# sloisel/MultiGridBarrierMPI.jl

Hardware: AMD Instinct MI355X
Metric: fem2d p-Laplace DoF/s per Newton step (higher is better)
Workload: dtype f64; 1 GPU; fem2d p-Laplace L=7 p=1 (n=57344 rows, N_L=49154 Newton unknowns), amgb main phase, tol=sqrt(eps); parallelism=single GPU

## Files before the change

multigridbarriermpi.jl_amd/csrc/gpuchol.hip:

```cpp
#include "gpuchol.hpp"

#include "amg.hpp"

#include <algorithm>
#include <array>
#include <cmath>
#include <cstdio>
#include <cstdlib>
#include <stdexcept>
#include <string>

namespace mgb {

namespace {

void ck(hipError_t e, const char* what) {
  if (e != hipSuccess) throw HipError(std::string("HIP error in gpuchol ") + what + ": " + hipGetErrorString(e));
}

constexpr int kProfSlots = 10;
#ifdef MGB_PROF_LAST_WG
#define MGB_PROF_WG (gridDim.x - 1)
#else
#define MGB_PROF_WG 0
// ... 980 lines not shown
      src[u] = (k < t.a1) ? asm_src[k] : 0;
    }
#pragma unroll
    for (int u = 0; u < 4; ++u) v[u] = vals[src[u]];
#pragma unroll
    for (int u = 0; u < 4; ++u) add_entry(pos[u], v[u]);
  }
  if (prm >= 0) ATI[tid * TP + nf - r0] += bval;
  __syncthreads();
  factor_diag_block<NARROW, DENSE>(D, kw, Lo, (t.ti == 0 && t.tj == 0) ? linv + t.loff : nullptr, fail, nullptr);
  if (!DENSE) {
    for (int idx = tid; idx < PB * PB; idx += TB) Lc[lq_index(idx % PB, idx / PB)] = Lo[(idx % PB) * LP + idx / PB];
    __syncthreads();
  }
  STAMP(2);
  const double* Lf = DENSE ? Lo : Lc;
  if (diag) trsm_block64<NARROW, DENSE>(ATI, TP, Lf, kw);
  else trsm_block64_pair<NARROW, DENSE>(ATI, ATJ, TP, Lf, kw);
  __syncthreads();
  if (t.tj == min((int)t.ti, max(1, (nf - k1 + TS - 1) / TS) - 1)) {
    for (int idx = tid; idx < TS * PB; idx += TB) {
      const int r = idx / PB, m = idx % PB;
      if (r0 + r <= nf && m < kw) F[(long long)ld * (r0 + r) + m] = ATI[m * TP + r];
    }
  }
  STAMP(3);
  if (PRE && DENSE) {
#pragma unroll
    for (int bj = 0; bj < 4; ++bj)
#pragma unroll
      for (int reg = 0; reg < 4; ++reg) {
        const int i = r0 + 16 * w + li, j = c0 + 16 * bj + lk + 4 * reg;
        c[bj][reg] = slab(i <= nf && j < nf && i >= j, i, j);
      }
  }
  typedef double v4f64 __attribute__((ext_vector_type(4)));
  const double* LI = ATI + 16 * w + li + lk * TP;
  const double* LJ = (diag ? ATI : ATJ) + li + lk * TP;
  v4f64 acc[4];
#pragma unroll
  for (int bj = 0; bj < 4; ++bj) acc[bj] = v4f64{c[bj][0], c[bj][1], c[bj][2], c[bj][3]};
#pragma unroll
  for (int ks = 0; ks < (NARROW ? 2 : PB / 4); ++ks) {
    const double bv = -LI[4 * ks * TP];
#pragma unroll
    for (int bj = 0; bj < 4; ++bj)
      acc[bj] = __builtin_amdgcn_mfma_f64_16x16x4f64(LJ[4 * ks * TP + 16 * bj], bv, acc[bj], 0, 0, 0);
  }
  double* E = slabs + (producer ? t.eoff : 0);
  const int* fwJ = rowJ[0];
  const int fi = producer ? rowI[0][16 * w + li] : 0;
#pragma unroll
  for (int bj = 0; bj < 4; ++bj)
#pragma unroll
    for (int reg = 0; reg < 4; ++reg) {
      const int i = r0 + 16 * w + li, j = c0 + 16 * bj + lk + 4 * reg;
      if (i <= nf && j < nf && i >= j) {
        if (producer) E[(long long)t.pld * fwJ[16 * bj + lk + 4 * reg] + fi] = acc[bj][reg];
        else F[(long long)ld * j + i] = acc[bj][reg];
      }
    }
  STAMP(7);
}

template <bool NARROW, bool PRE>
__global__ __launch_bounds__(TB) __attribute__((amdgpu_waves_per_eu(2, 2))) void front_single_kernel(
    const SingleTile* __restrict__ tiles, const int* __restrict__ pinv, const int* __restrict__ asm_src,
    const int* __restrict__ asm_pos, const double* __restrict__ vals, const int* __restrict__ perm, const double* __restrict__ b,
    const double* __restrict__ fronts_ro, double* fronts, double* linv, int* fail, long long* prof,
    const double* __restrict__ slabs_ro, double* slabs, const int* __restrict__ fwd) {
  front_single_body<NARROW, false, PRE>(tiles, pinv, asm_src, asm_pos, vals, perm, b, fronts_ro, fronts, linv, fail, prof, slabs_ro,
                                        slabs, fwd);
}

template <bool NARROW, bool PRE>
__global__ __launch_bounds__(TB) __attribute__((amdgpu_waves_per_eu(3, 3))) void front_single_dense_kernel(
    const SingleTile* __restrict__ tiles, const int* __restrict__ pinv, const int* __restrict__ asm_src,
    const int* __restrict__ asm_pos, const double* __restrict__ vals, const int* __restrict__ perm, const double* __restrict__ b,
    const double* __restrict__ fronts_ro, double* fronts, double* linv, int* fail, long long* prof,
    const double* __restrict__ slabs_ro, double* slabs, const int* __restrict__ fwd) {
  front_single_body<NARROW, true, PRE>(tiles, pinv, asm_src, asm_pos, vals, perm, b, fronts_ro, fronts, linv, fail, prof, slabs_ro,
                                       slabs, fwd);
}

__global__ __launch_bounds__(TB, 4) void front_leaf_kernel(
    const GNode* __restrict__ nodes, const int* __restrict__ list, const int* __restrict__ asm_src,
    const int* __restrict__ asm_pos, const double* __restrict__ vals, const int* __restrict__ perm,
    const double* __restrict__ b, double* fronts, double* linv, int* fail, long long* prof, double* slabs,
    const int* __restrict__ fwd) {
  extern __shared__ __attribute__((aligned(32))) double sm[];
  __shared__ int fw[TS];
  STAMP(0);
  const GNode nd = nodes[blockIdx.x];
  (void)list;
  const int nf = nd.nf, ld = nf + 1, ns = nd.ns, tid = threadIdx.x;
  const bool producer = nd.eoff >= 0;
  if (producer && tid <= nf - ns && tid < TS) fw[tid] = fwd[nd.fofs + tid];
  constexpr int TP = TS + 8;
  __shared__ __attribute__((aligned(32))) double fixed[TP * PB + PB * (PB + 1) / 2];
  double* Fs = sm;
  double* AT = fixed;
  double* D = fixed;
  double* Lo = fixed + TP * PB;
  auto P = [ld](int i, int j) { return j * ld - (j * (j - 1)) / 2 + (i - j); };
  const int total = nf * ld - (nf * (nf - 1)) / 2;
  double* F = fronts + nd.off;
  for (int idx = tid; idx < total; idx += TB) Fs[idx] = 0.0;
  __syncthreads();
  for (int k = nd.a0 + tid; k < nd.a1; k += TB) {
    const int pos = asm_pos[k], col = pos / ld;
    Fs[P(pos - col * ld, col)] += vals[asm_src[k]];
  }
  for (int c = tid; c < ns; c += TB) Fs[P(nf, c)] += b[perm[nd.first + c]];
  __syncthreads();
  STAMP(1);
  auto panel = [&](const int p) {
    const int k0 = p * PB, kw = min(PB, ns - k0), k1 = k0 + kw;
    for (int idx = tid; idx < PB * PB; idx += TB) {
      const int i = idx % PB, j = idx / PB;
      D[i * LP + j] = (i < kw && j <= i) ? Fs[P(k0 + i, k0 + j)] : 0.0;
    }
    __syncthreads();
    factor_diag_block<true, true>(D, kw, Lo, linv + nd.loff + (long long)p * 2 * PB * PB, fail, nullptr);
    for (int idx = tid; idx < TS * PB; idx += TB) {
      const int r = idx % TS, q = idx / TS;
      AT[q * TP + r] = (q < kw && k1 + r <= nf) ? Fs[P(k1 + r, k0 + q)] : 0.0;
    }
    __syncthreads();
    trsm_block64<true, true>(AT, TP, Lo, kw);
    __syncthreads();
    for (int idx = tid; idx < TS * PB; idx += TB) {
      const int r = idx / PB, m = idx % PB;
      if (k1 + r <= nf && m < kw) F[(long long)ld * (k1 + r) + k0 + m] = AT[m * TP + r];
    }
    typedef double v4f64 __attribute__((ext_vector_type(4)));
    const int lane = tid & 63, w = tid >> 6, li = lane & 15, lk = lane >> 4;
    const double* LI = AT + 16 * w + li + lk * TP;
    const double* LJ = AT + li + lk * TP;
    v4f64 acc[4];
#pragma unroll
    for (int bj = 0; bj < 4; ++bj) acc[bj] = v4f64{0.0, 0.0, 0.0, 0.0};
#pragma unroll 1
    for (int ks = 0; ks < (kw + 3) / 4; ++ks) {
      const double bv = LI[4 * ks * TP];
#pragma unroll
      for (int bj = 0; bj < 4; ++bj)
        acc[bj] = __builtin_amdgcn_mfma_f64_16x16x4f64(LJ[4 * ks * TP + 16 * bj], bv, acc[bj], 0, 0, 0);
    }
#pragma unroll
    for (int bj = 0; bj < 4; ++bj)
#pragma unroll
      for (int reg = 0; reg < 4; ++reg) {
        const int i = k1 + 16 * w + li, j = k1 + 16 * bj + lk + 4 * reg;
        if (i <= nf && j < nf && i >= j) Fs[P(i, j)] -= acc[bj][reg];
      }
    __syncthreads();
  };
  panel(0);
  if (ns > PB) panel(1);
  STAMP(2);
  const int nb = nf - ns;
  if (producer) {
    double* E = slabs + nd.eoff;
    for (int idx = tid; idx < (nb + 1) * nb; idx += TB) {
      const int a = idx % (nb + 1), q = idx / (nb + 1);
      if (a >= q) E[(long long)nd.pld * fw[q] + fw[a]] = Fs[P(ns + a, ns + q)];
    }
  } else {
    for (int idx = tid; idx < (nb + 1) * nb; idx += TB) {
      const int i = ns + idx % (nb + 1), j = ns + idx / (nb + 1);
      if (i >= j) F[(long long)ld * j + i] = Fs[P(i, j)];
    }
  }
  STAMP(7);
}

template <int NT>
__device__ inline void rect_part(const double* __restrict__ F, int ld, int ns, int nb, int j0, int jw,
                                 const double* xb, double* red, double* out , bool subtract) {
  const int tid = threadIdx.x;
  const int nsl = NT / jw, jl = tid % jw, sl = tid / jw, j = j0 + jl;
  double s = 0.0;
  if (sl < nsl && j < ns) {
    const double* col = F + (long long)ld * ns + j;
#pragma unroll 8
    for (int i = sl; i < nb; i += nsl) s = fma(col[(long long)ld * i], xb[i], s);
  }
  if (nsl > 1) {
    red[tid] = s;
    __syncthreads();
    if (sl == 0)
      for (int q = 1; q < nsl; ++q) s += red[q * jw + jl];
  }
  if (sl == 0 && j < ns) out[j] = subtract ? out[j] - s : s;
}

__global__ __launch_bounds__(RT) void backward_rect_kernel(const GNode* __restrict__ nodes, const RectJob* __restrict__ jobs,
                                                            const int* __restrict__ bdry_all,
                                                            const double* __restrict__ fronts, const double* __restrict__ y,
                                                            double* rect) {
  extern __shared__ double sh[];
  const RectJob job = jobs[blockIdx.x];
  const GNode nd = nodes[blockIdx.x];
  const int nf = nd.nf, ns = nd.ns, nb = nf - ns;
  const int* bd = bdry_all + nd.bofs;
  double* xb = sh;
  double* red = sh + nb;
  for (int i = threadIdx.x; i < nb; i += RT) xb[i] = y[bd[i]];
  __syncthreads();
  rect_part<RT>(fronts + nd.off, nf + 1, ns, nb, job.chunk * 64, 64, xb, red, rect + nd.first, false);
}

template <int NT>
__global__ __launch_bounds__(NT) void backward_kernel(const GNode* __restrict__ nodes, const int* __restrict__ list,
                                                       const int* __restrict__ bdry_all, const double* __restrict__ fronts,
                                                       const double* __restrict__ linv, const int* __restrict__ perm,
                                                       const double* __restrict__ rect, int use_rect, double* y, double* x,
                                                       long long* prof) {
  extern __shared__ double sh[];
  STAMP(0);
  const GNode nd = nodes[blockIdx.x];
  (void)list;
  const int nf = nd.nf, ns = nd.ns, nb = nf - ns, ld = nf + 1, tid = threadIdx.x;
  const double* F = fronts + nd.off;
  double* u = sh;
  double* xb = sh + ns;
  double* red = sh + nf;
  for (int i = tid; i < ns; i += NT) u[i] = F[(long long)ld * nf + i] - ((use_rect && nb > 0) ? rect[nd.first + i] : 0.0);
  STAMP(1);
  if (!use_rect && nb > 0) {
    const int* bd = bdry_all + nd.bofs;
    for (int i = tid; i < nb; i += NT) xb[i] = y[bd[i]];
    __syncthreads();
    const int jw = min(NT, (ns + 63) & ~63);
    for (int j0 = 0; j0 < ns; j0 += jw) {
      rect_part<NT>(F, ld, ns, nb, j0, jw, xb, red, u, true);
      __syncthreads();
    }
  }
  __syncthreads();
  STAMP(2);
  const int npanel = (ns + PB - 1) / PB;
  for (int pp = npanel - 1; pp >= 0; --pp) {
    const int k0 = pp * PB, kw = min(PB, ns - k0), k1 = k0 + kw;
    if (tid < 64) {
      const int c = tid & 31;
      const double* lpp = linv + nd.loff + (long long)pp * 2 * PB * PB + c;
      double lc[PB];
#pragma unroll
      for (int m = 0; m < PB; ++m) lc[m] = lpp[PB * m];
      double uc = (c < kw) ? u[k0 + c] : 0.0;
#pragma unroll
      for (int m = PB - 1; m >= 0; --m) {
        const double xm = readlane_f64(uc * lc[m], m);
        uc = (c == m) ? xm : fma(-lc[m], xm, uc);
      }
      if (tid < kw) u[k0 + c] = uc;
      if (pp == npanel - 1) STAMP(3);
    }
    __syncthreads();
    if (pp == npanel - 1) STAMP(4);
    if (k0 > 0) {
      const int jw = min(NT, (k0 + 63) & ~63), nsl = NT / jw;
      for (int jb = 0; jb < k0; jb += jw) {
        const int jl = tid % jw, sl = tid / jw, j = jb + jl;
        double s = 0.0;
        if (sl < nsl && j < k0) {
#pragma unroll 8
          for (int i = k0 + sl; i < k1; i += nsl) s = fma(F[(long long)ld * i + j], u[i], s);
        }
        if (nsl > 1) {
          red[tid] = s;
          __syncthreads();
          if (sl == 0)
            for (int q = 1; q < nsl; ++q) s += red[q * jw + jl];
        }
        if (sl == 0 && j < k0) u[j] -= s;
      }
      __syncthreads();
    }
    if (pp == npanel - 1) STAMP(5);
  }
  STAMP(6);
  for (int i = tid; i < ns; i += NT) {
    const double v = u[i];
    y[nd.first + i] = v;
    x[perm[nd.first + i]] = v;
  }
  STAMP(7);
}


__device__ __forceinline__ void load_pivot_block(double (&lc)[PB], const double* __restrict__ lpp, int lane) {
#pragma unroll
  for (int m = 0; m < PB; ++m) lc[m] = lpp[PB * m + (lane & 31)];
}

__device__ __forceinline__ void load_panel_rows(double (&f)[PB], const double* __restrict__ F, int ld, int k0, int kw, int jc) {
  const double* Fj = F + (long long)ld * k0 + max(min(jc, k0 - 1), 0);
#pragma unroll
  for (int r = 0; r < PB; ++r) f[r] = Fj[(long long)ld * min(r, kw - 1)];
}

__device__ __forceinline__ void panel_substitute(const double (&lc)[PB], double* up, int kw, int lane) {
  const int c = lane & 31;
  double uc = (c < kw) ? up[c] : 0.0;
#pragma unroll
  for (int m = PB - 1; m >= 0; --m) {
    const double xm = readlane_f64(uc * lc[m], m);
    uc = (c == m) ? xm : fma(-lc[m], xm, uc);
  }
  if (lane < kw) up[c] = uc;
}

template <int NSL>
__device__ __forceinline__ double panel_dot(const double (&f)[PB], const double* up, int kw) {
  double s[NSL];
#pragma unroll
  for (int q = 0; q < NSL; ++q) s[q] = 0.0;
#pragma unroll
  for (int r = 0; r < PB; ++r) {
    const double v = fma(f[r], up[min(r, kw - 1)], s[r % NSL]);
    s[r % NSL] = (r < kw) ? v : s[r % NSL];
  }
  double t = s[0];
#pragma unroll
  for (int q = 1; q < NSL; ++q) t += s[q];
  return t;
}

__device__ inline double panel_dot_any(const double* __restrict__ Fj, long long ld, const double* up, int kw, int nsl) {
  double t = 0.0;
  for (int q = 0; q < nsl; ++q) {
    double s = 0.0;
    for (int r = q; r < kw; r += nsl) s = fma(Fj[ld * r], up[r], s);
    t = q ? t + s : s;
  }
  return t;
}

__device__ __forceinline__ int uni(int v) { return __builtin_amdgcn_readfirstlane(v); }

__global__ __launch_bounds__(512) void backward_fused_kernel(const int* __restrict__ wgs, int wstride, int max_levels, int xs_cap,
                                                              int red_cap, const int* __restrict__ slots,
                                                              const double* __restrict__ fronts, const double* __restrict__ linv,
                                                              const int* __restrict__ perm, double* y, double* x, long long* prof) {
  extern __shared__ double sh[];
  STAMP(0);
  int* rec = (int*)sh;
  double* xs = sh + wstride / 2;
  double* red = xs + xs_cap;
  int* sl = (int*)(red + red_cap);
  const int tid = threadIdx.x, T = blockDim.x, W = T >> 6, wave = uni(tid >> 6), lane = tid & 63;
  {
    const int* src = wgs + (size_t)blockIdx.x * wstride;
    for (int i = tid; i < wstride; i += T) rec[i] = src[i];
  }
  __syncthreads();
  const int nlevels = rec[0], njobs = rec[1], first_lv = rec[2], sub_lv = rec[5];
  const int* jobs = rec + kFusedHdr + kFusedLevelInts * max_levels;
  for (int jb = wave; jb < njobs; jb += W) {
    const int* j = jobs + kFusedJobInts * jb;
    const int nf = uni(j[FJ_NF]), ns = uni(j[FJ_NS]), flags = uni(j[FJ_FLAGS]), base = uni(j[FJ_BASE]);
    const long long off = ((long long)uni(j[FJ_OFF + 1]) << 32) | (unsigned)uni(j[FJ_OFF]);
    const double* srcv = (flags & 2) ? y + uni(j[FJ_FIRST]) : fronts + off + (long long)(nf + 1) * nf;
    for (int i0 = 0; i0 < ns; i0 += 256) {
      double v[4];
#pragma unroll
      for (int k = 0; k < 4; ++k) {
        const int i = i0 + 64 * k + lane;
        v[k] = srcv[min(i, ns - 1)];
      }
#pragma unroll
      for (int k = 0; k < 4; ++k) {
        const int i = i0 + 64 * k + lane;
        if (i < ns) xs[base + i] = v[k];
      }
    }
    if (flags & 2) continue;
    const int nb = nf - ns;
    const int* ssrc = slots + uni(j[FJ_SOFS]);
    int* sdst = sl + uni(j[FJ_LSOFS]);
    for (int i0 = 0; i0 < nb; i0 += 256) {
      int v[4];
#pragma unroll
      for (int k = 0; k < 4; ++k) {
        const int i = i0 + 64 * k + lane;
        v[k] = ssrc[min(i, nb - 1)];
      }
#pragma unroll
      for (int k = 0; k < 4; ++k) {
        const int i = i0 + 64 * k + lane;
        if (i < nb) sdst[i] = v[k];
      }
    }
  }
  __syncthreads();
  STAMP(1);
  if (first_lv == sub_lv) STAMP(2);
  for (int lv = first_lv; lv < nlevels; ++lv) {
    const int* li = rec + kFusedHdr + kFusedLevelInts * lv;
    const int lofs = li[0], cnt = li[1], maxp = li[2], items = li[3];
    int G = W;
    while (G > 1 && W / G < cnt) G >>= 1;
    const int ngrp = W / G, GT = G << 6, grp = wave / G, gtid = tid - grp * GT, gw = wave - grp * G;
    double* redg = red + grp * items;
    for (int r0 = 0; r0 < cnt; r0 += ngrp) {
      const bool act = r0 + grp < cnt;
      const int* j = jobs + kFusedJobInts * (lofs + (act ? r0 + grp : 0));
      const int nf = uni(j[FJ_NF]), ns = uni(j[FJ_NS]), nsl = uni(j[FJ_NSL]), nt = uni(j[FJ_NT]), nb = nf - ns, ld = nf + 1;
      const long long off = ((long long)uni(j[FJ_OFF + 1]) << 32) | (unsigned)uni(j[FJ_OFF]);
      const long long loff = ((long long)uni(j[FJ_LOFF + 1]) << 32) | (unsigned)uni(j[FJ_LOFF]);
      const double* F = fronts + off;
      double* u = xs + uni(j[FJ_BASE]);
      const int npanel = (ns + PB - 1) / PB;
      const bool sub = act && gw == 0 && npanel > 0;
      double lc[PB], f[PB];
      if (sub) load_pivot_block(lc, linv + loff + (long long)(npanel - 1) * 2 * PB * PB, lane);
      if (items > 0) {
        if (act && nsl > 0) {
          const int* sj = sl + uni(j[FJ_LSOFS]);
          const int nit = ns * nsl, R = (nb + nsl - 1) / nsl;
          for (int it0 = gtid; it0 < nit; it0 += 2 * GT) {
            const int it1 = it0 + GT;
            const bool has1 = it1 < nit;
            const int q0 = it0 / ns, q1 = has1 ? it1 / ns : q0;
            const double* c0 = F + (long long)ld * ns + (it0 - q0 * ns);
            const double* c1 = F + (long long)ld * ns + (has1 ? it1 - q1 * ns : it0 - q0 * ns);
            double s0 = 0.0, s1 = 0.0;
            for (int r0 = 0; r0 < R; r0 += 8) {
              double a0[8], a1[8];
#pragma unroll
              for (int k = 0; k < 8; ++k) {
                a0[k] = c0[(long long)ld * min(q0 + (r0 + k) * nsl, nb - 1)];
                a1[k] = c1[(long long)ld * min(q1 + (r0 + k) * nsl, nb - 1)];
              }
#pragma unroll
              for (int k = 0; k < 8; ++k) {
                const int i0 = q0 + (r0 + k) * nsl, i1 = q1 + (r0 + k) * nsl;
                const double v0 = fma(a0[k], xs[sj[min(i0, nb - 1)]], s0), v1 = fma(a1[k], xs[sj[min(i1, nb - 1)]], s1);
                s0 = (i0 < nb) ? v0 : s0;
                s1 = (i1 < nb) ? v1 : s1;
              }
            }
            redg[it0] = s0;
            if (has1) redg[it1] = s1;
          }
        }
        __syncthreads();
        if (act && nsl > 0)
          for (int jc = gtid; jc < ns; jc += GT) {
            double s = redg[jc];
            for (int q = 1; q < nsl; ++q) s += redg[q * ns + jc];
            u[jc] = u[jc] - s;
          }
        __syncthreads();
      }
      if (act && npanel > 1) load_panel_rows(f, F, ld, (npanel - 1) * PB, ns - (npanel - 1) * PB, gtid);
      for (int it = 0; it < maxp; ++it) {
        const int pp = npanel - 1 - it, k0 = pp * PB, kw = min(PB, ns - k0);
        if (sub && pp >= 0) {
          panel_substitute(lc, u + k0, kw, lane);
          if (pp > 0) load_pivot_block(lc, linv + loff + (long long)(pp - 1) * 2 * PB * PB, lane);
        }
        __syncthreads();
        if (it == maxp - 1) break;
        if (act && pp > 0) {
          const int jw = min(nt, (k0 + 63) & ~63), nslp = nt / jw;
          for (int jc = gtid; jc < k0; jc += GT) {
            double s;
            if (jc >= GT) {
              s = panel_dot_any(F + (long long)ld * k0 + jc, ld, u + k0, kw, nslp);
            } else if (nslp == 1 || nslp == 2 || nslp == 4) {
              s = nslp == 1 ? panel_dot<1>(f, u + k0, kw) : nslp == 2 ? panel_dot<2>(f, u + k0, kw) : panel_dot<4>(f, u + k0, kw);
            } else {
              s = panel_dot_any(F + (long long)ld * k0 + jc, ld, u + k0, kw, nslp);
            }
            u[jc] -= s;
          }
          if (pp > 1) load_panel_rows(f, F, ld, k0 - PB, PB, gtid);
        }
        __syncthreads();
      }
      if (act && (uni(j[FJ_FLAGS]) & 1)) {
        const int first = uni(j[FJ_FIRST]);
        for (int i = gtid; i < ns; i += GT) {
          const double v = u[i];
          y[first + i] = v;
          x[perm[first + i]] = v;
        }
      }
    }
    if (lv + 1 == sub_lv) STAMP(2);
    if (lv >= sub_lv) STAMP(min(3 + lv - sub_lv, 6));
  }
  for (int k = 3 + nlevels - sub_lv; k < 7; ++k) STAMP(k);
  STAMP(7);
}

__global__ __launch_bounds__(256) void schur_pack_kernel(const RootXchg* __restrict__ roots, const double* __restrict__ fronts,
                                                         double* __restrict__ xb) {
  const RootXchg r = roots[blockIdx.x];
  const double* F = fronts + r.off;
  for (int j = blockIdx.y; j < r.nb; j += gridDim.y) {
    double* dst = xb + r.xoff + (long long)j * (r.nb + 1) - (long long)j * (j - 1) / 2 - j;
    const double* col = F + (long long)r.ld * (r.ns + j) + r.ns;
    for (int i = j + threadIdx.x; i <= r.nb; i += blockDim.x) dst[i] = r.owned ? col[i] : 0.0;
  }
}

__global__ __launch_bounds__(256) void schur_unpack_kernel(const RootXchg* __restrict__ roots, const double* __restrict__ xb,
                                                           double* __restrict__ fronts) {
  const RootXchg r = roots[blockIdx.x];
  double* F = fronts + r.off;
  for (int j = blockIdx.y; j < r.nb; j += gridDim.y) {
    const double* src = xb + r.xoff + (long long)j * (r.nb + 1) - (long long)j * (j - 1) / 2 - j;
    double* col = F + (long long)r.ld * (r.ns + j) + r.ns;
    for (int i = j + threadIdx.x; i <= r.nb; i += blockDim.x) col[i] = src[i];
  }
}

__global__ __launch_bounds__(256) void vals_pack_kernel(int n, const int* __restrict__ idx, const double* __restrict__ vals,
                                                        double* __restrict__ xb) {
  for (int i = blockIdx.x * blockDim.x + threadIdx.x; i < n; i += gridDim.x * blockDim.x) xb[i] = vals[idx[i]];
}

__global__ __launch_bounds__(256) void vals_unpack_kernel(int n, const int* __restrict__ idx, const double* __restrict__ xb,
                                                          double* __restrict__ vals) {
  for (int i = blockIdx.x * blockDim.x + threadIdx.x; i < n; i += gridDim.x * blockDim.x) vals[idx[i]] = xb[i];
}

__global__ __launch_bounds__(256) void xsol_pack_kernel(int n, const int* __restrict__ own, const double* __restrict__ x,
                                                        const int* __restrict__ fail, double* __restrict__ xs) {
  for (long long i = (long long)blockIdx.x * blockDim.x + threadIdx.x; i <= n; i += (long long)gridDim.x * blockDim.x)
    xs[i] = (i == n) ? (*fail ? 1.0 : 0.0) : (own[i] ? x[i] : 0.0);
}

__global__ __launch_bounds__(256) void x_local_kernel(int n, const int* __restrict__ kind, double* __restrict__ x) {
  for (long long i = (long long)blockIdx.x * blockDim.x + threadIdx.x; i < n; i += (long long)gridDim.x * blockDim.x)
    if (kind[i] == 0) x[i] = 0.0;
}

__global__ __launch_bounds__(256) void xsol_unpack_kernel(int n, const double* __restrict__ xs, double* __restrict__ x, int* fail) {
  for (long long i = (long long)blockIdx.x * blockDim.x + threadIdx.x; i <= n; i += (long long)gridDim.x * blockDim.x) {
    if (i == n) *fail = xs[n] != 0.0 ? 1 : 0;
    else x[i] = xs[i];
  }
}

}

template <class T>
T* GpuChol::upload(const std::vector<T>& v) {
  T* d = nullptr;
  const size_t bytes = std::max<size_t>(v.size(), 1) * sizeof(T);
  ck(hipMalloc((void**)&d, bytes), "hipMalloc");
  allocs_.push_back(d);
  if (!v.empty()) ck(hipMemcpy(d, v.data(), v.size() * sizeof(T), hipMemcpyHostToDevice), "H2D");
  return d;
}

GpuChol::~GpuChol() {
  for (GraphEntry& g : graphs_) (void)hipGraphExecDestroy(g.exec);
  for (void* p : allocs_) (void)hipFree(p);
}

const CholKnobs& GpuChol::knobs() {
  static const CholKnobs k = [] {
    auto on = [](const char* name) {
      const char* e = std::getenv(name);
      return !(e && e[0] == '0');
    };
    auto num = [](const char* name, int dflt) {
      const char* e = std::getenv(name);
      return e ? std::atoi(e) : dflt;
    };
    CholKnobs c;
    c.graph = on("MGB_CHOL_GRAPH");
    c.prof = std::getenv("MGB_CHOL_PROF") != nullptr;
    c.leaf = on("MGB_CHOL_LEAF");
    c.single = on("MGB_CHOL_SINGLE");
    c.step2 = on("MGB_CHOL_STEP2");
    c.wide = on("MGB_CHOL_WIDE");
    c.start_pivot = on("MGB_CHOL_START_PIVOT");
    c.step2_tiles = num("MGB_CHOL_STEP2_TILES", c.step2_tiles);
    c.dense_tiles = num("MGB_CHOL_DENSE_TILES", c.dense_tiles);
    c.bwd_split_nf = num("MGB_BWD_SPLIT_NF", c.bwd_split_nf);
    c.bwd_fused = on("MGB_CHOL_BWD_FUSED");
    c.bwd_cut = num("MGB_CHOL_BWD_CUT", c.bwd_cut);
    c.bwd_fused_nf = num("MGB_CHOL_BWD_FUSED_NF", c.bwd_fused_nf);
    c.bwd_fused_threads = num("MGB_CHOL_BWD_FUSED_THREADS", c.bwd_fused_threads);
    c.premap = num("MGB_CHOL_PREMAP", c.premap);
    c.premap_tiles = num("MGB_CHOL_PREMAP_TILES", c.premap_tiles);
    return c;
  }();
  return k;
}

void GpuChol::schedule_info(int cap, int* nlaunch, int* kind, int* workgroups) const {
  if (nlaunch) *nlaunch = (int)chain_.size();
  const int m = std::min(std::max(cap, 0), (int)chain_.size());
  for (int i = 0; i < m; ++i) {
    if (kind) kind[i] = (int)chain_[i].kind;
    if (workgroups) workgroups[i] = chain_[i].cnt;
  }
}

void GpuChol::premap_info(int cap, int* consumer, int* producers) const {
  const int m = std::min(std::max(cap, 0), (int)chain_.size());
  for (int i = 0; i < m; ++i) {
    if (consumer) consumer[i] = chain_[i].premap ? 1 : 0;
    if (producers) producers[i] = chain_[i].nproducers;
  }
}

void GpuChol::unknown_columns(const MfChol& sym, int* node, int* col) {
  const CholTree T = sym.view();
  for (int t = 0; t < T.size(); ++t)
    for (int k = 0; k < T.ns[t]; ++k) {
      const int i = (*T.perm)[T.first[t] + k];
      if (node) node[i] = t;
      if (col) col[i] = k;
    }
}

void GpuChol::build(const MfChol& sym, Ctx* ctx) {
  ctx_ = ctx;
  part_ = (ctx && ctx->world > 1) ? sym.partition(ctx->world) : CholPartition();
  const int my_rank = ctx ? ctx->rank : 0;
  const CholTree T = sym.view();
  ChainPlan P = plan_chain(T, part_, my_rank, knobs());
  const std::vector<GNode>& nodes = P.nodes;
  const std::vector<int>& perm = *T.perm;
  const int nnodes = T.size();
  n_ = T.n;
  flops_ = T.flops;
  total_front_ = T.front_doubles;
  chain_ = std::move(P.chain);
  own_bwd_ = P.own_bwd;
  top_fwd_ = P.top_fwd;
  premap_ = std::move(P.premap);
  fused_ = std::move(P.fused);
  d_nodes_ = upload(nodes);
  d_perm_ = upload(perm);
  d_bdry_ = upload(P.bdry);
  d_pinv_ = upload(premap_.pinv);
  d_fwd_ = upload(premap_.fwd);
  d_asm_src_ = upload(P.asrc);
  d_asm_pos_ = upload(P.apos);
  d_lists_ = upload(P.lists);
  {
    std::vector<GNode> hn(P.lists.size()), rn(P.rects.size());
    for (size_t k = 0; k < P.lists.size(); ++k) hn[k] = nodes[P.lists[k]];
    for (size_t k = 0; k < P.rects.size(); ++k) rn[k] = nodes[P.rects[k].node];
    d_hnodes_ = upload(hn);
    d_rnodes_ = upload(rn);
  }
  d_start_ = upload(P.starts);
  d_tiles_ = upload(P.tiles);
  d_singles_ = upload(P.singles);
  d_rectjobs_ = upload(P.rects);
  d_fused_wg_ = upload(fused_.wg);
  d_fused_slots_ = upload(fused_.slots);
  if (part_.split()) {
    std::vector<RootXchg> roots;
    long long xoff = 0;
    for (int j = 0; j < part_.world; ++j) {
      const GNode& g = nodes[part_.roots[j]];
      RootXchg r{};
      r.off = g.off;
      r.xoff = xoff;
      r.ld = g.nf + 1;
      r.ns = g.ns;
      r.nb = g.nf - g.ns;
      r.owned = (j == my_rank) ? 1 : 0;
      xoff += (long long)r.nb * (r.nb + 3) / 2;
      max_root_nb_ = std::max(max_root_nb_, r.nb);
      roots.push_back(r);
    }
    xchg_doubles_ = xoff;
    nroots_ = (int)roots.size();
    d_roots_ = upload(roots);
    std::vector<int> own(n_, 0);
    for (int t = 0; t < nnodes; ++t)
      if (part_.owner[t] == my_rank || (part_.owner[t] < 0 && my_rank == 0))
        for (int k = 0; k < nodes[t].ns; ++k) own[perm[nodes[t].first + k]] = 1;
    d_own_orig_ = upload(own);
    std::vector<int> kind(n_, 0), top_unk;
    for (int t = 0; t < nnodes; ++t)
      for (int k = 0; k < nodes[t].ns; ++k) {
        const int i = perm[nodes[t].first + k];
        kind[i] = part_.owner[t] < 0 ? 2 : (part_.owner[t] == my_rank ? 1 : 0);
        if (part_.owner[t] < 0) top_unk.push_back(i);
      }
    std::sort(top_unk.begin(), top_unk.end());
    d_kind_orig_ = upload(kind);
    ntop_unk_ = (int)top_unk.size();
    d_top_unk_ = upload(top_unk);
    vals_local_ = sym.rank_aligned(part_.world);
    if (vals_local_) {
      const std::vector<int> top_idx = sym.top_value_indices(part_);
      ntop_vals_ = (int)top_idx.size();
      d_top_idx_ = upload(top_idx);
    }
    ck(hipMalloc((void**)&d_xchg_, std::max<long long>(xchg_doubles_ + ntop_vals_, 1) * sizeof(double)), "hipMalloc xchg");
    allocs_.push_back(d_xchg_);
    ck(hipMalloc((void**)&d_xsol_, (size_t)(n_ + 1) * sizeof(double)), "hipMalloc xsol");
    allocs_.push_back(d_xsol_);
  }
  ck(hipMalloc((void**)&d_fronts_, std::max<long long>(total_front_, 1) * sizeof(double)), "hipMalloc fronts");
  allocs_.push_back(d_fronts_);
  ck(hipMemset(d_fronts_, 0, std::max<long long>(total_front_, 1) * sizeof(double)), "memset fronts");
  ck(hipMalloc((void**)&d_slabs_, std::max<long long>(premap_.slab_doubles, 1) * sizeof(double)), "hipMalloc slabs");
  allocs_.push_back(d_slabs_);
  ck(hipMemset(d_slabs_, 0, std::max<long long>(premap_.slab_doubles, 1) * sizeof(double)), "memset slabs");
  ck(hipMalloc((void**)&d_linv_, std::max<long long>(T.linv_doubles, 1) * sizeof(double)), "hipMalloc linv");
  allocs_.push_back(d_linv_);
  ck(hipMalloc((void**)&d_rect_, std::max(n_, 1) * sizeof(double)), "hipMalloc rect");
  allocs_.push_back(d_rect_);
  ck(hipMalloc((void**)&d_y_, std::max(n_, 1) * sizeof(double)), "hipMalloc y");
  allocs_.push_back(d_y_);
  ck(hipMalloc((void**)&d_fail_, sizeof(int)), "hipMalloc flag");
  allocs_.push_back(d_fail_);
  ck(hipMemset(d_fail_, 0, sizeof(int)), "memset");
  if (knobs().prof) {
    const size_t nl = chain_.size();
    ck(hipMalloc((void**)&d_prof_, kProfSlots * nl * sizeof(long long)), "hipMalloc prof");
    allocs_.push_back(d_prof_);
    reset_stamps();
#ifdef MGB_PROF_PER_WG
    {
      long long* wg = nullptr;
      ck(hipMalloc((void**)&wg, nl * kProfMaxWg * 2 * sizeof(long long)), "hipMalloc wgprof");
      allocs_.push_back(wg);
      ck(hipMemset(wg, 0, nl * kProfMaxWg * 2 * sizeof(long long)), "memset wgprof");
      ck(hipMemcpyToSymbol(HIP_SYMBOL(g_wgprof), &wg, sizeof(wg)), "symbol wgprof");
      ck(hipMemcpyToSymbol(HIP_SYMBOL(g_prof_base), &d_prof_, sizeof(d_prof_)), "symbol prof base");
      d_wgprof_ = wg;
    }
#endif
  }
  ck(hipFuncSetAttribute((const void*)backward_kernel<256>, hipFuncAttributeMaxDynamicSharedMemorySize, 150 * 1024), "attr");
  ck(hipFuncSetAttribute((const void*)backward_kernel<1024>, hipFuncAttributeMaxDynamicSharedMemorySize, 150 * 1024), "attr");
  ck(hipFuncSetAttribute((const void*)backward_rect_kernel, hipFuncAttributeMaxDynamicSharedMemorySize, 150 * 1024), "attr");
  ck(hipFuncSetAttribute((const void*)backward_fused_kernel, hipFuncAttributeMaxDynamicSharedMemorySize, 150 * 1024), "attr");
  ck(hipFuncSetAttribute((const void*)front_leaf_kernel, hipFuncAttributeMaxDynamicSharedMemorySize, 100 * 1024), "attr");
  ck(hipFuncSetAttribute((const void*)front_step2_kernel, hipFuncAttributeMaxDynamicSharedMemorySize, kStep2Lds), "attr");
  ck(hipFuncSetAttribute((const void*)front_panel2_kernel, hipFuncAttributeMaxDynamicSharedMemorySize, kPanel2Lds), "attr");
  ck(hipFuncSetAttribute((const void*)front_update2_kernel, hipFuncAttributeMaxDynamicSharedMemorySize, kUpdate2Lds), "attr");
}

void GpuChol::factor_solve(hipStream_t st, double* d_vals, const double* d_b, double* d_x, KernelTimer* tm, bool flag_armed,
                           bool values_summed, bool x_local) {
  if (n_ == 0) return;
  if (!flag_armed) ck(hipMemsetAsync(d_fail_, 0, sizeof(int), st), "memset flag");
  if (part_.split()) {
    factor_solve_split(st, d_vals, d_b, d_x, tm, values_summed, x_local && vals_local_ && !values_summed);
    return;
  }
  if (!knobs().graph || tm || d_prof_) {
    enqueue(st, d_vals, d_b, d_x, tm);
    return;
  }
  for (const GraphEntry& g : graphs_)
    if (g.vals == d_vals && g.b == d_b && g.x == d_x) {
      ck(hipGraphLaunch(g.exec, st), "hipGraphLaunch");
      return;
    }
  hipGraph_t graph = nullptr;
  ck(hipStreamBeginCapture(st, hipStreamCaptureModeThreadLocal), "hipStreamBeginCapture");
  try {
    enqueue(st, d_vals, d_b, d_x, nullptr);
  } catch (...) {
    (void)hipStreamEndCapture(st, &graph);
    if (graph) (void)hipGraphDestroy(graph);
    throw;
  }
  ck(hipStreamEndCapture(st, &graph), "hipStreamEndCapture");
  GraphEntry ge{d_vals, d_b, d_x, nullptr};
  ck(hipGraphInstantiate(&ge.exec, graph, nullptr, nullptr, 0), "hipGraphInstantiate");
  (void)hipGraphDestroy(graph);
  graphs_.push_back(ge);
  ck(hipGraphLaunch(ge.exec, st), "hipGraphLaunch");
}

namespace {
int timer_class(Kind k) {
  if (k <= Kind::SingleDenseNarrow) return KC_CHOL_SINGLE;
  if (k == Kind::Start) return KC_CHOL_START;
  if (k <= Kind::Update2) return KC_CHOL_STEP;
  return k == Kind::BwdRect ? KC_CHOL_BWD_RECT : KC_CHOL_BWD;
}
}

void GpuChol::run(hipStream_t st, int begin, int end, const double* d_vals, const double* d_b, double* d_x, KernelTimer* tm) {
  for (int i = begin; i < end; ++i) {
    const Launch& L = chain_[i];
    long long* prof = d_prof_ ? d_prof_ + (size_t)kProfSlots * i : nullptr;
    const dim3 grid(L.cnt), block(L.block);
// ... 160 lines not shown
```

Measured before the change: 90.25 million DoF/s per Newton step.

## Add lookahead pipelining to fused backward panel substitution and defer output writes

Restructures the backward triangular solve in the fused kernel. When multiple waves cooperate, the substituting wave now updates the next panel's rows from register-held solution values via readlane before solving that panel, while the other waves update the remaining rows in parallel. The aim is to shorten the serial critical path of panel substitution. Output writes for upper-level jobs are moved to a single pass at the end of the kernel. This adds complexity and a separate code path whose correctness relies on careful synchronization.

New measurement: 91.45 million DoF/s per Newton step, median of 6. 1.3% higher.

```diff
diff --git a/multigridbarriermpi.jl_amd/csrc/gpuchol.hip b/multigridbarriermpi.jl_amd/csrc/gpuchol.hip
--- a/multigridbarriermpi.jl_amd/csrc/gpuchol.hip
+++ b/multigridbarriermpi.jl_amd/csrc/gpuchol.hip
@@ -1306,7 +1306,7 @@
   for (int r = 0; r < PB; ++r) f[r] = Fj[(long long)ld * min(r, kw - 1)];
 }
 
-__device__ __forceinline__ void panel_substitute(const double (&lc)[PB], double* up, int kw, int lane) {
+__device__ __forceinline__ double panel_substitute(const double (&lc)[PB], double* up, int kw, int lane) {
   const int c = lane & 31;
   double uc = (c < kw) ? up[c] : 0.0;
 #pragma unroll
@@ -1315,6 +1315,7 @@
     uc = (c == m) ? xm : fma(-lc[m], xm, uc);
   }
   if (lane < kw) up[c] = uc;
+  return uc;
 }
 
 template <int NSL>
@@ -1326,6 +1327,23 @@
   for (int r = 0; r < PB; ++r) {
     const double v = fma(f[r], up[min(r, kw - 1)], s[r % NSL]);
     s[r % NSL] = (r < kw) ? v : s[r % NSL];
+  }
+  double t = s[0];
+#pragma unroll
+  for (int q = 1; q < NSL; ++q) t += s[q];
+  return t;
+}
+
+template <int NSL>
+__device__ __forceinline__ double panel_dot_lanes(const double (&f)[PB], double xq, int kw) {
+  double s[NSL];
+#pragma unroll
+  for (int q = 0; q < NSL; ++q) s[q] = 0.0;
+#pragma unroll
+  for (int r = 0; r < PB; ++r) {
+    const double v = fma(f[r], readlane_f64(xq, r), s[r % NSL]);
+    s[r % NSL] = (r < kw) ? v : s[r % NSL];
+    if (r % 8 == 7) __builtin_amdgcn_sched_barrier(0);
   }
   double t = s[0];
 #pragma unroll
@@ -1341,6 +1359,28 @@
     t = q ? t + s : s;
   }
   return t;
+}
+
+__device__ __forceinline__ double panel_update(const double (&f)[PB], bool in_f, const double* __restrict__ Fj, long long ld,
+                                               const double* up, int kw, int nslp) {
+  if (in_f && nslp == 1) return panel_dot<1>(f, up, kw);
+  if (in_f && nslp == 2) return panel_dot<2>(f, up, kw);
+  if (in_f && nslp == 4) return panel_dot<4>(f, up, kw);
+  return panel_dot_any(Fj, ld, up, kw, nslp);
+}
+
+__device__ __forceinline__ void lookahead_step(double (&lc)[PB], double (&f)[PB], double& xq, const double* __restrict__ F, int ld,
+                                               int ns, int nt, int q0, double* u, const double* __restrict__ lnext, int lane) {
+  const int k0 = q0 - PB, qw = min(PB, ns - q0), jc = k0 + (lane & 31);
+  const int jw = min(nt, (q0 + 63) & ~63), nslp = nt / jw;
+  const double s = nslp == 1   ? panel_dot_lanes<1>(f, xq, qw)
+                   : nslp == 2 ? panel_dot_lanes<2>(f, xq, qw)
+                   : nslp == 4 ? panel_dot_lanes<4>(f, xq, qw)
+                               : panel_dot_any(F + (long long)ld * q0 + jc, ld, u + q0, qw, nslp);
+  if (lane < PB) u[jc] -= s;
+  load_panel_rows(f, F, ld, k0, PB, k0 - PB + (lane & 31));
+  xq = panel_substitute(lc, u + k0, PB, lane);
+  load_pivot_block(lc, lnext, lane);
 }
 
 __device__ __forceinline__ int uni(int v) { return __builtin_amdgcn_readfirstlane(v); }
@@ -1460,33 +1500,40 @@
           }
         __syncthreads();
       }
-      if (act && npanel > 1) load_panel_rows(f, F, ld, (npanel - 1) * PB, ns - (npanel - 1) * PB, gtid);
-      for (int it = 0; it < maxp; ++it) {
-        const int pp = npanel - 1 - it, k0 = pp * PB, kw = min(PB, ns - k0);
-        if (sub && pp >= 0) {
-          panel_substitute(lc, u + k0, kw, lane);
-          if (pp > 0) load_pivot_block(lc, linv + loff + (long long)(pp - 1) * 2 * PB * PB, lane);
+      const bool lead = sub && G > 1 && npanel > 1;
+      if (lead) {
+        int k0 = (npanel - 1) * PB;
+        load_panel_rows(f, F, ld, k0, ns - k0, k0 - PB + (lane & 31));
+        double xq = panel_substitute(lc, u + k0, ns - k0, lane);
+        load_pivot_block(lc, linv + loff + (long long)(npanel - 2) * 2 * PB * PB, lane);
+        __syncthreads();
+        for (int pp = npanel - 2; pp >= 0; --pp) {
+          lookahead_step(lc, f, xq, F, ld, ns, nt, k0, u, linv + loff + (long long)max(pp - 1, 0) * 2 * PB * PB, lane);
+          k0 -= PB;
+          __syncthreads();
         }
-        __syncthreads();
-        if (it == maxp - 1) break;
-        if (act && pp > 0) {
-          const int jw = min(nt, (k0 + 63) & ~63), nslp = nt / jw;
-          for (int jc = gtid; jc < k0; jc += GT) {
-            double s;
-            if (jc >= GT) {
-              s = panel_dot_any(F + (long long)ld * k0 + jc, ld, u + k0, kw, nslp);
-            } else if (nslp == 1 || nslp == 2 || nslp == 4) {
-              s = nslp == 1 ? panel_dot<1>(f, u + k0, kw) : nslp == 2 ? panel_dot<2>(f, u + k0, kw) : panel_dot<4>(f, u + k0, kw);
-            } else {
-              s = panel_dot_any(F + (long long)ld * k0 + jc, ld, u + k0, kw, nslp);
+        for (int it = npanel; it < maxp; ++it) __syncthreads();
+      } else {
+        const int OT = G > 1 ? GT - 64 : GT, ot = G > 1 ? gtid - 64 : gtid;
+        if (act && npanel > 1) load_panel_rows(f, F, ld, (npanel - 1) * PB, ns - (npanel - 1) * PB, ot);
+        for (int it = 0; it < maxp; ++it) {
+          const int pp = npanel - 1 - it, k0 = pp * PB, kw = min(PB, ns - k0), q0 = k0 + PB, qw = min(PB, ns - q0);
+          if (act && pp >= 0) {
+            if (it > 0) {
+              const int jw = min(nt, (q0 + 63) & ~63), nslp = nt / jw, hi = G > 1 ? k0 : q0;
+              for (int jc = ot; jc < hi; jc += OT)
+                u[jc] -= panel_update(f, jc < OT, F + (long long)ld * q0 + jc, ld, u + q0, qw, nslp);
+              if (hi > PB) load_panel_rows(f, F, ld, k0, PB, ot);
             }
-            u[jc] -= s;
+            if (sub) {
+              panel_substitute(lc, u + k0, kw, lane);
+              if (pp > 0) load_pivot_block(lc, linv + loff + (long long)(pp - 1) * 2 * PB * PB, lane);
+            }
           }
-          if (pp > 1) load_panel_rows(f, F, ld, k0 - PB, PB, gtid);
+          __syncthreads();
         }
-        __syncthreads();
-      }
-      if (act && (uni(j[FJ_FLAGS]) & 1)) {
+      }
+      if (lv >= sub_lv && act && (uni(j[FJ_FLAGS]) & 1)) {
         const int first = uni(j[FJ_FIRST]);
         for (int i = gtid; i < ns; i += GT) {
           const double v = u[i];
@@ -1499,6 +1546,19 @@
     if (lv >= sub_lv) STAMP(min(3 + lv - sub_lv, 6));
   }
   for (int k = 3 + nlevels - sub_lv; k < 7; ++k) STAMP(k);
+  const int npath = sub_lv < nlevels ? rec[kFusedHdr + kFusedLevelInts * sub_lv] : njobs;
+  __syncthreads();
+  for (int jb = wave; jb < npath; jb += W) {
+    const int* j = jobs + kFusedJobInts * jb;
+    if (!(uni(j[FJ_FLAGS]) & 1)) continue;
+    const int ns = uni(j[FJ_NS]), first = uni(j[FJ_FIRST]);
+    const double* u = xs + uni(j[FJ_BASE]);
+    for (int i = lane; i < ns; i += 64) {
+      const double v = u[i];
+      y[first + i] = v;
+      x[perm[first + i]] = v;
+    }
+  }
   STAMP(7);
 }
 
```
